# shijun18/H-DenseFormer

Measured on AMD Instinct MI355X. Metric: train samples/sec on 4x128^3 volumes, higher is better.
Workload: dtype bf16

## Files before the change

### h-denseformer_amd/csrc/conv_igemm.hip

```cpp
#include "conv_igemm.h"
#include "conv_tile.h"
#include <type_traits>

namespace {

template <typename T, int TD, int TH, int TW, int WM, int WN, int MB, int S, bool CONVT, bool FLAT = false>
__global__ __launch_bounds__(256, (FLAT && S == 1) ? 3 : 2) void conv_igemm_kernel(ConvArgs a) {
  if (a.prio) HDF_LIGHT_PRIO();
  static_assert(WM * WN == 4, "4 waves");
  static_assert(WM * MB * 32 == TD * TH * TW, "tile/wave decomposition");
  static_assert(!FLAT || TD == 1, "flat tiles are one voxel deep");
  constexpr int BD = FLAT ? 1 : (CONVT ? TD + 1 : S * (TD - 1) + 3);
  constexpr int BH = CONVT ? TH + 1 : S * (TH - 1) + 3;
  constexpr int BW = CONVT ? TW + 1 : S * (TW - 1) + 3;
  constexpr int SS = CONVT ? 1 : S;
  constexpr int ESZ = sizeof(T);
  __shared__ __attribute__((aligned(16))) char lds[BD * BH * BW * PITCH + 4 * 32 * 2 * 4];
  float* s_red = reinterpret_cast<float*>(lds + BD * BH * BW * PITCH);

  const int lane = threadIdx.x & 63, wave = threadIdx.x >> 6;
  const int r = lane & 31, h = lane >> 5;
  const int wm = wave / WN, wn = wave % WN;

  const int Td = CONVT ? a.Di : a.Do, Th = CONVT ? a.Hi : a.Ho, Tw = CONVT ? a.Wi : a.Wo;
  const int ntz = (Td + TD - 1) / TD, nty = (Th + TH - 1) / TH, ntx = (Tw + TW - 1) / TW;
  int t = blockIdx.x;
  const int tx = t % ntx;
  t /= ntx;
  const int ty = t % nty;
  t /= nty;
  const int tz = t % ntz;
  const int n = t / ntz;
  const int z0 = tz * TD, y0 = ty * TH, x0 = tx * TW;
  const int n_base = blockIdx.y * (WN * 32) + wn * 32;
  const int cls = CONVT ? blockIdx.z : 0;
  const int pz = FLAT ? 0 : (cls >> 2) & 1, py = (cls >> 1) & 1, px = cls & 1;
  const int ntapz = FLAT ? 1 : (CONVT ? (pz ? 2 : 1) : 3), ntapy = CONVT ? (py ? 2 : 1) : 3, ntapx = CONVT ? (px ? 2 : 1) : 3;

  const int oz = (CONVT || FLAT) ? z0 : S * z0 - 1, oy = CONVT ? y0 : S * y0 - 1, ox = CONVT ? x0 : S * x0 - 1;

  constexpr bool ZXMAP = !CONVT && !FLAT && S == 1 && TD == 4 && TW == 8 && WM * MB == TH && (2 * BH * BW) % 16 == 8;
  constexpr bool YXMAP = FLAT && SS == 1 && TW == 16 && 2 * WM * MB == TH;
  auto mrow_voxel = [](int mblk, int row, int& lz, int& ly, int& lx) {
    if constexpr (ZXMAP) {
      ws_row_to_zx(row, lz, lx);
      ly = mblk;
    } else if constexpr (YXMAP) {
      int g2;
      ds128_group(row, g2, lx);
      lz = 0;
      ly = 2 * mblk + g2;
    } else {
      const int lin = mblk * 32 + row;
      lz = lin / (TH * TW), ly = (lin / TW) % TH, lx = lin % TW;
    }
  };
  int rowbase[MB];
#pragma unroll
  for (int mb = 0; mb < MB; mb++) {
    int lz, ly, lx;
    mrow_voxel(wm * MB + mb, r, lz, ly, lx);
    rowbase[mb] = (((FLAT ? 0 : SS * lz)) * BH + SS * ly) * BW + SS * lx;
  }
  const bool n_active = n_base < a.CoutP;
  const char* wrow = reinterpret_cast<const char*>(a.w) + ((int64_t)(n_base + r) * a.Cin) * ESZ + h * 16;
  const int64_t wtap_stride = (int64_t)a.CoutP * a.Cin * ESZ;
  const int chunk_elems_max = 64 / ESZ;

  const char* const wfr = a.wfrag ? reinterpret_cast<const char*>(a.w) +
                                        (int64_t)(n_base >> 5) * ((a.Cin * ESZ) >> 5) * 1024 + r * 32 + h * 16
                                  : wrow;
  const int cstride = a.wfrag ? 2048 : 64, fstride = a.wfrag ? 1024 : 32;

  bool done = false;
  f32x16 acc[MB];
#pragma unroll
  for (int mb = 0; mb < MB; mb++)
#pragma unroll
    for (int i = 0; i < 16; i++) acc[mb][i] = 0.f;
  if constexpr (!CONVT) {
    if ((a.Cin * ESZ) % 64 == 0) {
      constexpr int NS = FLAT ? 18 : 54;
      constexpr int TAP0 = FLAT ? 9 : 0;
      constexpr int V1_RING_BIG = 6, V1_RING_SMALL = 9;
      constexpr int RING = (MB >= 4) ? V1_RING_BIG : V1_RING_SMALL;
      const int nchunk_all = a.Cin * ESZ / 64;
      const int kz = a.ksplit > 1 ? (int)blockIdx.z : 0;
      const int c_lo = a.ksplit > 1 ? kz * (nchunk_all / a.ksplit) : 0;
      const int nchunk = a.ksplit > 1 ? c_lo + nchunk_all / a.ksplit : nchunk_all;
      u32x4 bq[RING];
      auto b_load = [&](int chunk, int s_) -> u32x4 {
        const int tap = TAP0 + (s_ >> 1), fs = s_ & 1;
        const char* p = wfr + tap * wtap_stride + (int64_t)chunk * cstride + fs * fstride;
        return *reinterpret_cast<const u32x4*>(n_active ? p : reinterpret_cast<const char*>(a.w));
      };
      auto a_off = [&](int s_) {
        const int tap = s_ >> 1, fs = s_ & 1;
        return ((tap / 9 * BH + (tap / 3) % 3) * BW + tap % 3) * PITCH + h * 16 + fs * 32;
      };
#pragma unroll
      for (int k = 0; k < RING; k++) bq[k] = b_load(c_lo, k);
      for (int chunk = c_lo; chunk < nchunk; chunk++) {
        if (chunk > c_lo) __syncthreads();
        stage_box<T, BD, BH, BW, 64, PITCH>(lds, reinterpret_cast<const T*>(a.in), a.in_pitch, a.Cin, n, a.Di, a.Hi,
                                            a.Wi, oz, oy, ox, chunk * chunk_elems_max, 64, a.in_scale, a.in_shift,
                                            a.in_relu);
        __syncthreads();
        u32x4 af[2][MB];
#pragma unroll
        for (int mb = 0; mb < MB; mb++) af[0][mb] = *reinterpret_cast<const u32x4*>(lds + rowbase[mb] * PITCH + a_off(0));
        const bool more = chunk + 1 < nchunk;
#pragma unroll
        for (int s_ = 0; s_ < NS; s_++) {
          if (s_ + 1 < NS) {
#pragma unroll
            for (int mb = 0; mb < MB; mb++)
              af[(s_ + 1) & 1][mb] = *reinterpret_cast<const u32x4*>(lds + rowbase[mb] * PITCH + a_off(s_ + 1));
          }
          const u32x4 bcur = bq[s_ % RING];
          __builtin_amdgcn_sched_barrier(0);
#pragma unroll
          for (int mb = 0; mb < MB; mb++) Mma<T>::run(af[s_ & 1][mb], bcur, acc[mb]);
          if (s_ + RING < NS)
            bq[s_ % RING] = b_load(chunk, s_ + RING);
          else if (more)
            bq[s_ % RING] = b_load(chunk + 1, s_ + RING - NS);
          __builtin_amdgcn_sched_barrier(0);
        }
      }
      done = true;
    }
  }
  for (int c0 = 0; !done && c0 < a.Cin; c0 += chunk_elems_max) {
    const int chunk_elems = min(chunk_elems_max, a.Cin - c0);
    const int row_bytes = chunk_elems * ESZ;
    if (c0 > 0) __syncthreads();
    stage_box<T, BD, BH, BW, 64, PITCH>(lds, reinterpret_cast<const T*>(a.in), a.in_pitch, a.Cin, n, a.Di, a.Hi, a.Wi,
                                        oz, oy, ox, c0, row_bytes, a.in_scale, a.in_shift, a.in_relu);
    __syncthreads();
    if (n_active) {
      const int nfs = row_bytes >> 5;
      for (int jz = 0; jz < ntapz; jz++) {
        const int offz = FLAT ? 0 : (CONVT ? (pz ? 1 - jz : 0) : jz), wz = FLAT ? 1 : (CONVT ? (pz ? 2 * jz : 1) : jz);
        for (int jy = 0; jy < ntapy; jy++) {
          const int offy = CONVT ? (py ? 1 - jy : 0) : jy, wy = CONVT ? (py ? 2 * jy : 1) : jy;
#pragma unroll
          for (int jx = 0; jx < 3; jx++) {
            if (jx < ntapx) {
              const int offx = CONVT ? (px ? 1 - jx : 0) : jx, wx = CONVT ? (px ? 2 * jx : 1) : jx;
              const int tapoff = ((offz * BH + offy) * BW + offx) * PITCH + h * 16;
              const char* wp = wfr + ((wz * 3 + wy) * 3 + wx) * wtap_stride + (int64_t)(c0 * ESZ / 64) * cstride;
              for (int fs = 0; fs < nfs; fs++) {
                u32x4 bfrag = *reinterpret_cast<const u32x4*>(wp + fs * fstride);
                u32x4 afrag[MB];
#pragma unroll
                for (int mb = 0; mb < MB; mb++)
                  afrag[mb] = *reinterpret_cast<const u32x4*>(lds + rowbase[mb] * PITCH + tapoff + fs * 32);
#pragma unroll
                for (int mb = 0; mb < MB; mb++) Mma<T>::run(afrag[mb], bfrag, acc[mb]);
              }
            }
          }
        }
      }
    }
  }

  const int ch = n_base + r;
  if constexpr (!CONVT) {
    if (a.ksplit > 1) {
      if (n_active) {
        const int64_t mtot = (int64_t)a.N * a.Do * a.Ho * a.Wo;
#pragma unroll
        for (int mb = 0; mb < MB; mb++) {
#pragma unroll
          for (int i = 0; i < 16; i++) {
            const int row = (i & 3) + 8 * (i >> 2) + 4 * h;
            int lz, ly, lx;
            mrow_voxel(wm * MB + mb, row, lz, ly, lx);
            const int gz = z0 + lz, gy = y0 + ly, gx = x0 + lx;
            if (gz < Td && gy < Th && gx < Tw)
              a.kpart[((int64_t)blockIdx.z * mtot + (((int64_t)n * a.Do + gz) * a.Ho + gy) * a.Wo + gx) * a.CoutP + ch] =
                  acc[mb][i];
          }
        }
      }
      return;
    }
  }
  const bool ch_ok = n_active && ch < a.Cout;
  const float bias = (a.bias && ch_ok) ? a.bias[ch] : 0.f;
  float s1 = 0.f, s2 = 0.f;
  T* outp = (a.split && n_base >= a.split) ? reinterpret_cast<T*>(a.out2) - a.split : reinterpret_cast<T*>(a.out);
#pragma unroll
  for (int mb = 0; mb < MB; mb++) {
    float old[16];
    if (a.accumulate) {
#pragma unroll
      for (int i = 0; i < 16; i++) {
        int row = (i & 3) + 8 * (i >> 2) + 4 * h;
        int lz, ly, lx;
        mrow_voxel(wm * MB + mb, row, lz, ly, lx);
        int gz = z0 + lz, gy = y0 + ly, gx = x0 + lx;
        const bool ok = ch_ok && gz < Td && gy < Th && gx < Tw;
        int qz = (CONVT && !FLAT) ? 2 * gz + pz : gz, qy = CONVT ? 2 * gy + py : gy, qx = CONVT ? 2 * gx + px : gx;
        const T* p = outp + ((((int64_t)n * a.Do + qz) * a.Ho + qy) * a.Wo + qx) * a.out_pitch + ch;
        old[i] = ST<T>::ld(ok ? p : outp);
      }
    } else {
#pragma unroll
      for (int i = 0; i < 16; i++) old[i] = 0.f;
    }
#pragma unroll
    for (int i = 0; i < 16; i++) {
      int row = (i & 3) + 8 * (i >> 2) + 4 * h;
      int lz, ly, lx;
      mrow_voxel(wm * MB + mb, row, lz, ly, lx);
      int gz = z0 + lz, gy = y0 + ly, gx = x0 + lx;
      if (ch_ok && gz < Td && gy < Th && gx < Tw) {
        int qz = (CONVT && !FLAT) ? 2 * gz + pz : gz, qy = CONVT ? 2 * gy + py : gy, qx = CONVT ? 2 * gx + px : gx;
        T* p = outp + ((((int64_t)n * a.Do + qz) * a.Ho + qy) * a.Wo + qx) * a.out_pitch + ch;
        float v = acc[mb][i] + bias + old[i];
        ST<T>::st(p, v);
        s1 += v;
        s2 += v * v;
      }
    }
  }
  if (a.stat_partials) {
    s1 += __shfl_xor(s1, 32, 64);
    s2 += __shfl_xor(s2, 32, 64);
    __syncthreads();
    if (h == 0) {
      s_red[((wm * WN + wn) * 32 + r) * 2 + 0] = s1;
      s_red[((wm * WN + wn) * 32 + r) * 2 + 1] = s2;
    }
    __syncthreads();
    if (threadIdx.x < WN * 32) {
      int c = blockIdx.y * (WN * 32) + threadIdx.x;
      if (c < a.CoutP) {
        float t1 = 0.f, t2 = 0.f;
#pragma unroll
        for (int k = 0; k < WM; k++) {
          t1 += s_red[(k * WN * 32 + threadIdx.x) * 2 + 0];
          t2 += s_red[(k * WN * 32 + threadIdx.x) * 2 + 1];
        }
        float* q = a.stat_partials + ((int64_t)blockIdx.x * a.CoutP + c) * 2;
        q[0] = t1;
        q[1] = t2;
      }
    }
  }
}

template <int CH>
__device__ __forceinline__ int a_swz(int row) {
  return CH == 64 ? ((row >> 2) & 3) : ((row >> 3) & 1);
}

template <typename T, int CH, int RB, bool XF, int NB, bool BS = false, int TDP = 4>
__global__ __launch_bounds__(256) void conv_ws2_kernel(ConvArgs a) {
  if (a.prio) HDF_LIGHT_PRIO();
  constexpr int TD = TDP, ZH = TDP / 4, TH = 8, TW = 8, BD = TD + 2, BH = TH + 2, BW = TW + 2, BOX = BD * BH * BW;
  static_assert(TDP == 4 || TDP == 8, "tile depth");
  constexpr int ESZ = sizeof(T), EPC = ST<T>::EPC;
  constexpr int CIN = RB / ESZ;
  constexpr int NCH = RB / CH, NFS = CH / 32, NG = 9 * NFS;
  constexpr int CPV = CH / 16, CPV_SHIFT = (CPV == 4) ? 2 : 1;
  constexpr int TOTAL = BOX * CPV, NJ = (TOTAL + 255) / 256;
  constexpr bool SWZ = (2 * BOX * (CH + 16) + 4096 + 512 + 27 * 32 * NB * RB > 160 * 1024);
  constexpr int AP = SWZ ? CH : CH + 16;
  constexpr int ABUF = BOX * AP;
  constexpr int OFF_RED = 2 * ABUF, OFF_XF = OFF_RED + 2048 * NB, OFF_W = OFF_XF + 512;
  constexpr int NC = 32 * NB;
  constexpr int CPR = RB / 16, RP256 = 16 / CPR;
  static_assert(CH == 32 || CH == 64, "chunk bytes");
  static_assert(NCH == 1 || NCH % 2 == 0, "buffer parity at tile start must be compile-time");
  static_assert(2 * CIN * 4 <= 512, "scale/shift table");
  static_assert(OFF_W + 27 * NC * RB <= 160 * 1024, "LDS budget");
  static_assert(ZH == 1 || !SWZ, "the 8-deep tile needs the padded layout");
  __shared__ __attribute__((aligned(256))) char lds[OFF_W + 27 * NC * RB];
#ifdef WS_DBG_STAMPS
  const unsigned long long t_entry = __builtin_amdgcn_s_memrealtime();
#endif
  char* const a_lds = lds;
  float* const s_red = reinterpret_cast<float*>(lds + OFF_RED);
  float* const s_xf = reinterpret_cast<float*>(lds + OFF_XF);
  char* const w_lds = lds + OFF_W;

  const int tid = threadIdx.x, lane = tid & 63, wave = tid >> 6;
  const int r = lane & 31, h = lane >> 5;
  const int n0 = blockIdx.y * NC;
  const int part = tid & (CPV - 1);
  constexpr bool xf = XF;
  const float relu_lo = (xf && a.in_relu) ? 0.f : -INFINITY;

  {
    constexpr int WTOT = 27 * NC * CPR, WIT = (WTOT + 255) / 256;
    u32x4 wv[WIT];
    const int rot = blockIdx.x % WIT;
#pragma unroll
    for (int u = 0; u < WIT; u++) {
      int it = u + rot;
      it -= (it >= WIT) ? WIT : 0;
      const int id = min(tid + 256 * it, WTOT - 1);
      const int row = id / CPR, ch = id - row * CPR;
      const int tap = row / NC, rr = row - tap * NC;
      wv[u] = *reinterpret_cast<const u32x4*>(reinterpret_cast<const char*>(a.w) +
                                             ((int64_t)(tap * a.CoutP + n0 + rr) * CIN) * ESZ + ch * 16);
    }
#pragma unroll
    for (int u = 0; u < WIT; u++) {
      int it = u + rot;
      it -= (it >= WIT) ? WIT : 0;
      const int id = tid + 256 * it;
      const int row = id / CPR, ch = id - row * CPR;
      const int sw = ch ^ ((row / RP256) & (CPR - 1));
      if (id < WTOT) *reinterpret_cast<u32x4*>(w_lds + row * RB + sw * 16) = wv[u];
    }
  }
  const int bswz = (r / RP256) & (CPR - 1);

  const int ntz = (a.Do + TD - 1) / TD, nty = (a.Ho + TH - 1) / TH, ntx = (a.Wo + TW - 1) / TW;
  const bool has_int = ntz >= 3 && nty >= 3 && ntx >= 3;
  const int ipz = ntz - 2, ipy = nty - 2, ipx = ntx - 2;
  const int n_int = has_int ? a.N * ipz * ipy * ipx : 0;
  const int per_all = ntz * nty * ntx, per_bor = per_all - (has_int ? ipz * ipy * ipx : 0);
  const int n_bor = a.N * per_bor;
  const int G = gridDim.x;
  const int NX = (G % 8 == 0) ? 8 : 1;
  const int WPX = G / NX;
  const int xcd = blockIdx.x % NX, slot = blockIdx.x / NX;
  auto split = [&](int total, int& begin, int& cnt) {
    const int r0 = (int)((int64_t)total * xcd / NX), r1 = (int)((int64_t)total * (xcd + 1) / NX);
    begin = r0 + slot;
    cnt = (r1 - r0 > slot) ? (r1 - r0 - slot + WPX - 1) / WPX : 0;
  };
  int int_begin, int_cnt, bor_begin, bor_cnt;
  split(n_int, int_begin, int_cnt);
  split(n_bor, bor_begin, bor_cnt);
  if (int_cnt + bor_cnt == 0) return;
  int sdx = 0, sdy = 0, sdz = 0, sdn = 0;
  if (has_int) {
    int t = WPX;
    sdx = t % ipx, t /= ipx;
    sdy = t % ipy, t /= ipy;
    sdz = t % ipz, sdn = t / ipz;
  }

  int aaddr[SWZ ? 3 : 1][SWZ ? 4 : 1][SWZ ? 3 : 1];
  int abase;
  {
    int dz, x;
    ws_row_to_zx(r, dz, x);
    abase = ((dz * BH + 2 * wave) * BW + x) * AP + h * 16;
    if constexpr (SWZ) {
#pragma unroll
      for (int jz = 0; jz < 3; jz++)
#pragma unroll
        for (int yp = 0; yp < 4; yp++)
#pragma unroll
          for (int jx = 0; jx < 3; jx++) {
            int row = ((dz + jz) * BH + 2 * wave + yp) * BW + x + jx;
            aaddr[jz][yp][jx] = row * CH + ((h ^ a_swz<CH>(row)) << 4);
          }
    }
  }
  auto a_addr = [&](int jz, int yp, int jx, int fs, int zh = 0) {
    if constexpr (SWZ)
      return aaddr[jz][yp][jx] ^ (fs * 32);
    else
      return abase + (((jz + 4 * zh) * BH + yp) * BW + jx) * AP + fs * 32;
  };
  int bvar[NCH];
#pragma unroll
  for (int c = 0; c < NCH; c++) bvar[c] = r * RB + (((c * CPV + h) ^ bswz) << 4);
  int boff[NJ], bxyz[NJ], woff_t[SWZ ? NJ : 2];
#pragma unroll
  for (int j = 0; j < NJ; j++) {
    int vox = min(tid + 256 * j, TOTAL - CPV + part) >> CPV_SHIFT;
    int bz = vox / (BH * BW), rem = vox - bz * (BH * BW), by = rem / BW, bx = rem - by * BW;
    boff[j] = ((bz * a.Hi + by) * a.Wi + bx) * (int)a.in_pitch;
    bxyz[j] = (bz << 16) | (by << 8) | bx;
    if constexpr (SWZ) {
      woff_t[j] = vox * CH + ((part ^ a_swz<CH>(vox)) << 4);
    } else {
      if (j == 0) woff_t[0] = vox * AP + part * 16;
      if (j == NJ - 1) woff_t[1] = vox * AP + part * 16;
    }
  }
  auto woff = [&](int j) {
    if constexpr (SWZ)
      return woff_t[j];
    else
      return j == NJ - 1 ? woff_t[1] : woff_t[0] + j * (256 / CPV) * AP;
  };

  auto tile_lin = [&](const WsTile& c) { return ((c.n * ntz + c.z0 / TD) * nty + (c.y0 >> 3)) * ntx + (c.x0 >> 3); };
  auto int_init = [&](WsTile& c, int k) {
    int t = k;
    c.x0 = (t % ipx + 1) * TW;
    t /= ipx;
    c.y0 = (t % ipy + 1) * TH;
    t /= ipy;
    c.z0 = (t % ipz + 1) * TD;
    c.n = t / ipz;
    c.tile = tile_lin(c);
  };
  auto int_next = [&](WsTile& c) {
    int xi = (c.x0 >> 3) - 1 + sdx, yi = (c.y0 >> 3) - 1 + sdy, zi = c.z0 / TD - 1 + sdz;
    c.n += sdn;
    if (xi >= ipx) xi -= ipx, yi++;
    if (yi >= ipy) yi -= ipy, zi++;
    if (zi >= ipz) zi -= ipz, c.n++;
    c.x0 = (xi + 1) * TW, c.y0 = (yi + 1) * TH, c.z0 = (zi + 1) * TD;
    c.tile = tile_lin(c);
  };
  auto bor_init = [&](WsTile& c, int k) {
    int tz, ty, tx;
    c.k = k;
    c.n = k / per_bor;
    int rem = k - c.n * per_bor;
    if (!has_int) {
      tx = rem % ntx, ty = (rem / ntx) % nty, tz = rem / (ntx * nty);
    } else {
      const int plane = nty * ntx, ring = plane - ipy * ipx;
      if (rem < plane) {
        tz = 0, ty = rem / ntx, tx = rem % ntx;
      } else if (rem - plane < ipz * ring) {
        rem -= plane;
        tz = 1 + rem / ring;
        rem %= ring;
        if (rem < ntx) {
          ty = 0, tx = rem;
        } else if (rem - ntx < 2 * ipy) {
          rem -= ntx;
          ty = 1 + (rem >> 1), tx = (rem & 1) ? ntx - 1 : 0;
        } else {
          ty = nty - 1, tx = rem - ntx - 2 * ipy;
        }
      } else {
        rem -= plane + ipz * ring;
        tz = ntz - 1, ty = rem / ntx, tx = rem % ntx;
      }
    }
    c.z0 = tz * TD, c.y0 = ty * TH, c.x0 = tx * TW;
    c.tile = tile_lin(c);
  };
  auto bor_next = [&](WsTile& c) { bor_init(c, c.k + WPX); };
  auto tile_interior = [&](const WsTile& c) {
    return c.z0 >= 1 && c.y0 >= 1 && c.x0 >= 1 && c.z0 + TD + 1 <= a.Di && c.y0 + TH + 1 <= a.Hi &&
           c.x0 + TW + 1 <= a.Wi;
  };
  const T* const src_safe = reinterpret_cast<const T*>(a.in) + part * EPC;
  auto tile_org = [&](const WsTile& c) -> const T* {
    return src_safe + ((((int64_t)c.n * a.Di + (c.z0 - 1)) * a.Hi + (c.y0 - 1)) * a.Wi + (c.x0 - 1)) * a.in_pitch;
  };

  u32x4 pf[NJ];
  auto slot_ok = [&](int j, const WsTile& c) {
    int iz = c.z0 - 1 + (bxyz[j] >> 16), iy = c.y0 - 1 + ((bxyz[j] >> 8) & 255), ix = c.x0 - 1 + (bxyz[j] & 255);
    return ((unsigned)iz < (unsigned)a.Di) & ((unsigned)iy < (unsigned)a.Hi) & ((unsigned)ix < (unsigned)a.Wi);
  };
  auto load_one = [&](auto fast_tag, int j, int chunk, const WsTile& c, bool valid, bool inter, const T* org) {
    if constexpr (decltype(fast_tag)::value) {
      pf[j] = *reinterpret_cast<const u32x4*>(org + boff[j] + chunk * (CH / ESZ));
    } else {
      const bool ok = inter | (valid & slot_ok(j, c));
      const T* p = ok ? org + boff[j] + chunk * (CH / ESZ) : src_safe;
      pf[j] = *reinterpret_cast<const u32x4*>(p);
    }
  };
  float sc[EPC], sh[EPC];
  auto read_xf = [&](int chunk) {
    const int cb = chunk * (CH / ESZ) + part * EPC;
#pragma unroll
    for (int e = 0; e < EPC; e += 4) {
      f32x4 u = *reinterpret_cast<const f32x4*>(s_xf + cb + e);
      f32x4 v = *reinterpret_cast<const f32x4*>(s_xf + CIN + cb + e);
#pragma unroll
      for (int k = 0; k < 4; k++) {
        sc[e + k] = u[k];
        sh[e + k] = v[k];
      }
    }
  };
  auto commit_one = [&](auto fast_tag, int j, const WsTile& c, bool inter, char* dst) {
    u32x4 v = pf[j];
    if constexpr (XF) {
      float f[EPC];
      ST<T>::unpack(v, f);
#pragma unroll
      for (int e = 0; e < EPC; e++) f[e] = fmaxf(f[e] * sc[e] + sh[e], relu_lo);
      v = ST<T>::pack(f);
    }
    if constexpr (!decltype(fast_tag)::value) {
      const bool ok = inter | slot_ok(j, c);
#pragma unroll
      for (int k = 0; k < 4; k++) v[k] = ok ? v[k] : 0u;
    }
    *reinterpret_cast<u32x4*>(dst + woff(j)) = v;
  };
  int tbl_n = -1;
  auto refresh_xf = [&](int n) {
    if (tid < CIN) {
      s_xf[tid] = xf ? a.in_scale[(int64_t)n * CIN + tid] : 1.f;
      s_xf[CIN + tid] = xf ? a.in_shift[(int64_t)n * CIN + tid] : 0.f;
    }
    tbl_n = n;
    __syncthreads();
  };

  WsTile T0, T1, T2;
  bool v1 = false, v2 = false, i0 = false, i1 = false, i2 = false;
  const T *org0 = src_safe, *org1 = src_safe, *org2 = src_safe;
  int left = 0;
  auto begin_pass = [&](auto border_tag, int k, int count) __attribute__((always_inline)) {
    constexpr bool BORDER = decltype(border_tag)::value;
    auto next = [&](WsTile& c) {
      if constexpr (BORDER)
        bor_next(c);
      else
        int_next(c);
    };
    if constexpr (BORDER)
      bor_init(T0, k);
    else
      int_init(T0, k);
    left = count - 1;
    T1 = T0;
    next(T1);
// ... 149 lines not shown
              const float g = (yv[mb][i] * bsc + bsh > 0.f) ? ST<T>::ld(&tmp) : 0.f;
              s1 += g;
              s2 += g * ((yv[mb][i] - bmu) * brs);
            }
          }
          }
        } else {
#pragma unroll
        for (int zh = 0; zh < ZH; zh++)
#pragma unroll
        for (int mb = 0; mb < 2; mb++) {
          T* const orow = obase + (int64_t)mb * a.Wo * a.out_pitch + zh * ezh;
#pragma unroll
          for (int i = 0; i < 16; i++) {
            const float v = acc[(nb * ZH + zh) * 2 + mb][i] + bias[nb];
            ST<T>::st(orow + eoff(i), v);
            s1 += v;
            s2 += v * v;
          }
        }
        }
      } else if (full && ch_ok[nb]) {
#pragma unroll
        for (int zh = 0; zh < ZH; zh++)
#pragma unroll
        for (int mb = 0; mb < 2; mb++) {
          T* const orow = obase + (int64_t)mb * a.Wo * a.out_pitch + zh * ezh;
          float old[16];
#pragma unroll
          for (int i = 0; i < 16; i++) old[i] = ST<T>::ld(orow + eoff(i));
#pragma unroll
          for (int i = 0; i < 16; i++) {
            const float v = acc[(nb * ZH + zh) * 2 + mb][i] + bias[nb];
            ST<T>::st(orow + eoff(i), v + old[i]);
            s1 += v;
            s2 += v * v;
          }
        }
      } else {
#pragma unroll
        for (int zh = 0; zh < ZH; zh++)
#pragma unroll
        for (int mb = 0; mb < 2; mb++) {
          const int gy = y0 + 2 * wave + mb;
          T* const orow = obase + (int64_t)mb * a.Wo * a.out_pitch + zh * ezh;
#pragma unroll
          for (int i = 0; i < 16; i++) {
            const int gz = z0 + edz[i >> 2] + 4 * zh, gx = x0 + (i & 3) + 4 * ((i >> 2) & 1);
            const float v = acc[(nb * ZH + zh) * 2 + mb][i] + bias[nb];
            const bool ok = gz < a.Do && gy < a.Ho && gx < a.Wo;
            if (ok && ch_ok[nb]) {
              float o = v;
              if (a.accumulate) o += ST<T>::ld(orow + eoff(i));
              ST<T>::st(orow + eoff(i), o);
            }
            const float mk = ok ? 1.f : 0.f;
            s1 += mk * v;
            s2 += mk * v * v;
          }
        }
      }
      if (PLAIN || ch_ok[nb]) {
        lr1[nb] += s1;
        lr2[nb] += s2;
      }
    }
  };

  f32x16 acc[2 * NB * ZH];
  auto tile_phase = [&](auto par_tag, auto fast_tag, auto plain_tag) __attribute__((always_inline)) {
    constexpr int PAR0 = decltype(par_tag)::value;
#pragma unroll
    for (int c = 0; c < NCH; c++) {
      constexpr int dummy = 0;
      (void)dummy;
      const int PAR = (PAR0 + c) & 1;
      char* const a_rd = a_lds + PAR * ABUF;
      char* const a_wr = a_lds + (1 - PAR) * ABUF;
      const bool c_next = (c + 1 >= NCH);
      const int c_chunk = (c + 1) % NCH;
      const int l_tile = (c + 2) / NCH;
      const int l_chunk = (c + 2) % NCH;
      const WsTile& CT = c_next ? T1 : T0;
      const bool c_int = c_next ? (i1 | !v1) : i0;
      const WsTile& LT = l_tile == 0 ? T0 : (l_tile == 1 ? T1 : T2);
      const bool l_val = l_tile == 0 ? true : (l_tile == 1 ? v1 : v2);
      const bool l_int = l_tile == 0 ? i0 : (l_tile == 1 ? i1 : i2);
      const T* const l_org = l_tile == 0 ? org0 : (l_tile == 1 ? org1 : org2);
      WS2_STAMP(3)
      if constexpr (XF) {
        if (CT.n != tbl_n && (!c_next || v1)) refresh_xf(CT.n);
        read_xf(c_chunk);
      }
      WS2_STAMP(0)
      u32x4 af[2][4 * ZH], bf[2][3 * NB];
      const char* w_rd = w_lds;
      if constexpr (RB == 32) asm volatile("" : "+v"(w_rd));
      auto read_group = [&](int g, u32x4 (&A)[4 * ZH], u32x4 (&B)[3 * NB]) {
        const int t = g / NFS, fs = g % NFS, jz = t / 3, jx = t % 3;
        auto rdA = [&](int yp) {
#pragma unroll
          for (int zh = 0; zh < ZH; zh++) A[zh * 4 + yp] = *reinterpret_cast<const u32x4*>(a_rd + a_addr(jz, yp, jx, fs, zh));
        };
        auto rdB = [&](int jy) {
#pragma unroll
          for (int nb = 0; nb < NB; nb++)
            B[jy * NB + nb] = *reinterpret_cast<const u32x4*>(w_rd + ((jz * 9 + jy * 3 + jx) * NC + 32 * nb) * RB +
                                                              (bvar[c] ^ (fs * 32)));
        };
        rdB(0);
        rdA(0);
        rdA(1);
        rdB(1);
        rdA(2);
        rdB(2);
        rdA(3);
      };
      read_group(0, af[0], bf[0]);
#pragma unroll
      for (int g = 0; g < NG; g++) {
        if (g + 1 < NG) read_group(g + 1, af[(g + 1) & 1], bf[(g + 1) & 1]);
        __builtin_amdgcn_sched_barrier(0);
#pragma unroll
        for (int j = 0; j < NJ; j++) {
          if ((j * NG) / NJ == g) {
            commit_one(fast_tag, j, CT, c_int, a_wr);
            load_one(fast_tag, j, l_chunk, LT, l_val, l_int, l_org);
          }
        }
        u32x4(&A)[4 * ZH] = af[g & 1];
        u32x4(&B)[3 * NB] = bf[g & 1];
        if (c == 0 && g == 0) {
#pragma unroll
          for (int q2 = 0; q2 < 2 * NB * ZH; q2++)
#pragma unroll
            for (int i = 0; i < 16; i++) acc[q2][i] = 0.f;
        }
#pragma unroll
        for (int jy = 0; jy < 3; jy++)
#pragma unroll
          for (int nb = 0; nb < NB; nb++)
#pragma unroll
            for (int zh = 0; zh < ZH; zh++) {
              Mma<T>::run(A[zh * 4 + jy], B[jy * NB + nb], acc[(nb * ZH + zh) * 2 + 0]);
              Mma<T>::run(A[zh * 4 + jy + 1], B[jy * NB + nb], acc[(nb * ZH + zh) * 2 + 1]);
            }
        __builtin_amdgcn_sched_barrier(0);
      }
      WS2_STAMP(1)
      WS_BARRIER();
      WS2_STAMP(2)
    }
    epilogue(acc, T0, plain_tag);
    WS2_STAMP(4)
  };

  using P0 = std::integral_constant<int, 0>;
  using P1 = std::integral_constant<int, 1>;
  using Yes = std::true_type;
  using No = std::false_type;
  bool more = true;
  auto step = [&](auto border_tag) __attribute__((always_inline)) {
    constexpr bool BORDER = decltype(border_tag)::value;
    more = v1;
    if (!more) return;
    left--;
    T0 = T1;
    T1 = T2;
    i0 = i1;
    i1 = i2;
    v1 = v2;
    org0 = org1;
    org1 = org2;
    if constexpr (BORDER)
      bor_next(T2);
    else
      int_next(T2);
    v2 = left >= 2;
    i2 = v2 && (BORDER ? tile_interior(T2) : true);
    org2 = v2 ? tile_org(T2) : src_safe;
  };

  if (int_cnt > 0) {
    begin_pass(No{}, int_begin, int_cnt);
    more = true;
    int par = 0;
    if (plain) {
      while (more) {
        if (NCH > 1 || par == 0)
          tile_phase(P0{}, Yes{}, Yes{});
        else
          tile_phase(P1{}, Yes{}, Yes{});
        if (NCH == 1) par ^= 1;
        step(No{});
      }
    } else {
      while (more) {
        if (NCH > 1 || par == 0)
          tile_phase(P0{}, Yes{}, No{});
        else
          tile_phase(P1{}, Yes{}, No{});
        if (NCH == 1) par ^= 1;
        step(No{});
      }
    }
  }
  if (bor_cnt > 0) {
    begin_pass(Yes{}, bor_begin, bor_cnt);
    stats_to_row();
    cur_pass = 1;
    more = true;
    int par = 0;
    while (more) {
      if (NCH > 1 || par == 0)
        tile_phase(P0{}, No{}, No{});
      else
        tile_phase(P1{}, No{}, No{});
      if (NCH == 1) par ^= 1;
      step(Yes{});
    }
  }
  stats_to_row();
#ifdef WS_DBG_STAMPS
  if (tid == 0 && blockIdx.y == 0) {
    for (int k = 0; k < 5; k++) a.stat_partials[(int64_t)blockIdx.x * 8 + k] = (float)tacc[k];
    a.stat_partials[(int64_t)blockIdx.x * 8 + 5] = __uint_as_float((uint32_t)treal0);
    a.stat_partials[(int64_t)blockIdx.x * 8 + 6] = __uint_as_float((uint32_t)__builtin_amdgcn_s_memrealtime());
    a.stat_partials[(int64_t)blockIdx.x * 8 + 7] = (float)(__builtin_amdgcn_s_memtime() - tcyc0);
    a.stat_partials[2048 + blockIdx.x] = __uint_as_float((uint32_t)t_entry);
  }
#endif
}

template <typename T, int TD, int TH, int TW>
__global__ __launch_bounds__(256) void conv_ksplit_reduce_kernel(ConvArgs a) {
  if (a.prio) HDF_LIGHT_PRIO();
  __shared__ float red[16][64][2];
  const int ntz = (a.Do + TD - 1) / TD, nty = (a.Ho + TH - 1) / TH, ntx = (a.Wo + TW - 1) / TW;
  int t = blockIdx.x;
  const int tx = t % ntx;
  t /= ntx;
  const int ty = t % nty;
  t /= nty;
  const int tz = t % ntz, n = t / ntz;
  const int cl = ((int)threadIdx.x & 15) * 4, c0 = blockIdx.y * 64 + cl, vl = (int)threadIdx.x >> 4;
  const bool c_on = c0 < a.CoutP;
  const int64_t mtot = (int64_t)a.N * a.Do * a.Ho * a.Wo;
  float bias[4], s1[4] = {0.f, 0.f, 0.f, 0.f}, s2[4] = {0.f, 0.f, 0.f, 0.f};
#pragma unroll
  for (int e = 0; e < 4; e++) bias[e] = (a.bias && c0 + e < a.Cout) ? a.bias[c0 + e] : 0.f;
  constexpr int TV = TD * TH * TW, IT = (TV + 15) / 16;
  static_assert(TV % 16 == 0, "tile voxels per voxel lane");
  if (c_on) {
#pragma unroll 2
    for (int it = 0; it < IT; it++) {
      const int lin = vl + 16 * it;
      const int gz = tz * TD + lin / (TH * TW), gy = ty * TH + (lin / TW) % TH, gx = tx * TW + lin % TW;
      const bool ok = gz < a.Do && gy < a.Ho && gx < a.Wo;
      const int64_t vox = ok ? (((int64_t)n * a.Do + gz) * a.Ho + gy) * a.Wo + gx : 0;
      f32x4 pv[4];
#pragma unroll
      for (int k = 0; k < 4; k++)
        pv[k] = *reinterpret_cast<const f32x4*>(a.kpart + ((int64_t)min(k, a.ksplit - 1) * mtot + vox) * a.CoutP + c0);
      f32x4 v = pv[0];
      for (int k = 1; k < a.ksplit; k++) v += pv[k];
      if (ok) {
        T* p = reinterpret_cast<T*>(a.out) + vox * a.out_pitch + c0;
#pragma unroll
        for (int e = 0; e < 4; e++) {
          if (c0 + e < a.Cout) {
            float o = v[e] + bias[e];
            if (a.accumulate) o += ST<T>::ld(p + e);
            ST<T>::st(p + e, o);
            s1[e] += o;
            s2[e] += o * o;
          }
        }
      }
    }
  }
  if (a.stat_partials) {
#pragma unroll
    for (int e = 0; e < 4; e++) red[vl][cl + e][0] = s1[e], red[vl][cl + e][1] = s2[e];
    __syncthreads();
    if (threadIdx.x < 128) {
      const int c = threadIdx.x >> 1, j = threadIdx.x & 1;
      if (blockIdx.y * 64 + c < a.CoutP) {
        float sum = 0.f;
#pragma unroll
        for (int k = 0; k < 16; k++) sum += red[k][c][j];
        a.stat_partials[((int64_t)blockIdx.x * a.CoutP + blockIdx.y * 64 + c) * 2 + j] = sum;
      }
    }
  }
}

template <typename T, int TD, int TH, int TW, int WM, int WN, int MB, int S, bool CONVT, bool FLAT = false>
int launch_cfg(const ConvArgs& a0, hipStream_t st) {
  ConvArgs a = a0;
  const int Td = CONVT ? a.Di : a.Do, Th = CONVT ? a.Hi : a.Ho, Tw = CONVT ? a.Wi : a.Wo;
  const int tiles = a.N * ceil_div(Td, TD) * ceil_div(Th, TH) * ceil_div(Tw, TW), nblk = ceil_div(a.CoutP, WN * 32);
  a.ksplit = 1;
  if constexpr (!CONVT && S == 1) {
    const int nchunk = (a.Cin * (int)sizeof(T)) % 64 == 0 ? a.Cin * (int)sizeof(T) / 64 : 0;
    if (a.kpart && !a.split && a.CoutP <= 1024 && a.CoutP % 4 == 0 && a.out_pitch % 4 == 0) {
      for (int ks = 4; ks >= 2; ks >>= 1) {
        const size_t need = (size_t)ks * a.N * a.Do * a.Ho * a.Wo * a.CoutP * sizeof(float);
        if (tiles * nblk * ks <= hdf_cu_budget() && nchunk % ks == 0 && nchunk / ks >= 2 && need <= a.kpart_bytes) {
          a.ksplit = ks;
          break;
        }
      }
    }
  }
  dim3 grid(tiles, nblk, CONVT ? (FLAT ? 4 : 8) : a.ksplit);
  hipLaunchKernelGGL((conv_igemm_kernel<T, TD, TH, TW, WM, WN, MB, S, CONVT, FLAT>), grid, dim3(256), 0, st, a);
  HDF_LAUNCH_CHECK();
  if constexpr (!CONVT && S == 1) {
    if (a.ksplit > 1) {
      hipLaunchKernelGGL((conv_ksplit_reduce_kernel<T, TD, TH, TW>), dim3(tiles, ceil_div(a.CoutP, 64)), dim3(256), 0, st, a);
      HDF_LAUNCH_CHECK();
    }
  }
  return HDF_OK;
}

inline bool small_tile(int Do, int Ho, int Wo) {
  return (int64_t)Do * Ho * Wo <= 32 * 32 * 32 / 2;
}
inline bool tiny_tile(int Do, int Ho, int Wo) {
  return (int64_t)Do * Ho * Wo <= 8 * 8 * 16;
}
inline int ws_cfg(int mode, int Do, int Ho, int Wo, int row_bytes) {
  if (mode != 0 || row_bytes > 128 || (int64_t)Do * Ho * Wo < 48 * 48 * 48 || Do == 1) return 0;
  return (row_bytes == 32 || row_bytes == 64 || row_bytes == 128) ? 1 : 0;
}

template <typename T, int CH, int RB, int NB>
int launch_ws2(const ConvArgs& a, hipStream_t st) {
  const int budget = a.cu_budget > 0 ? std::min(a.cu_budget, hdf_cu_budget()) : hdf_cu_budget();
  const int cout_tiles = a.CoutP / (32 * NB);
#ifndef HDF_NO_WS2_TD8
  if constexpr (sizeof(T) == 2 && NB == 1 && RB == 64) {
    if (a.in_scale && !a.bs_y && a.Do % 8 == 0 && a.Do >= 24 && a.Ho >= 24 && a.Wo >= 24) {
      const int tiles8 = a.N * (a.Do / 8) * ceil_div(a.Ho, 8) * ceil_div(a.Wo, 8);
      const int gx8 = std::min(tiles8, std::max(1, budget / cout_tiles));
      hipLaunchKernelGGL((conv_ws2_kernel<T, CH, RB, true, NB, false, 8>), dim3(gx8, cout_tiles), dim3(256), 0, st, a);
      HDF_LAUNCH_CHECK();
      return HDF_OK;
    }
  }
#endif
  const int tiles = a.N * ceil_div(a.Do, 4) * ceil_div(a.Ho, 8) * ceil_div(a.Wo, 8);
  const int gx = std::min(tiles, std::max(1, budget / cout_tiles));
  if constexpr (sizeof(T) == 2 && NB == 1 && RB == 64) {
    if (a.bs_y && !a.in_scale) {
      hipLaunchKernelGGL((conv_ws2_kernel<T, CH, RB, false, NB, true>), dim3(gx, cout_tiles), dim3(256), 0, st, a);
      HDF_LAUNCH_CHECK();
      return HDF_OK;
    }
  }
  HDF_CHECK_ARG(a.bs_y == nullptr, "conv: backward statistics are not available for this launch (hdf_conv_bwd_stats_ok)");
  if (a.in_scale)
    hipLaunchKernelGGL((conv_ws2_kernel<T, CH, RB, true, NB>), dim3(gx, cout_tiles), dim3(256), 0, st, a);
  else
    hipLaunchKernelGGL((conv_ws2_kernel<T, CH, RB, false, NB>), dim3(gx, cout_tiles), dim3(256), 0, st, a);
  HDF_LAUNCH_CHECK();
  return HDF_OK;
}

inline int flat_tile(int Ho, int Wo) { return (int64_t)Ho * Wo <= 32 * 32 ? 0 : ((int64_t)Ho * Wo <= 64 * 64 ? 1 : 2); }

template <typename T>
int launch_conv_t(int mode, const ConvArgs& a, hipStream_t st) {
  if (a.Di == 1) {
    HDF_CHECK_ARG(a.Do == 1 && !a.bs_y, "conv: a depth-1 input selects the 2-D operator (output depth 1, no statistics epilogue of the 3-D data gradient)");
    if (mode == 0) {
      const int ft = flat_tile(a.Ho, a.Wo);
      if (ft == 0) return launch_cfg<T, 1, 8, 8, 2, 2, 1, 1, false, true>(a, st);
      if (ft == 1) return launch_cfg<T, 1, 8, 16, 2, 2, 2, 1, false, true>(a, st);
      if (a.CoutP <= 32) return launch_cfg<T, 1, 16, 16, 4, 1, 2, 1, false, true>(a, st);
      return launch_cfg<T, 1, 16, 16, 2, 2, 4, 1, false, true>(a, st);
    } else if (mode == 1) {
      if (a.CoutP <= 64) return launch_cfg<T, 1, 8, 8, 2, 2, 1, 2, false, true>(a, st);
      return launch_cfg<T, 1, 8, 8, 1, 4, 2, 2, false, true>(a, st);
    } else {
      if (hdf_convt_fused_takes(ST<T>::DT, a)) return hdf_launch_convt_fused(ST<T>::DT, a, st);
      if (a.CoutP <= 32) return launch_cfg<T, 1, 16, 16, 4, 1, 2, 1, true, true>(a, st);
      return launch_cfg<T, 1, 8, 16, 2, 2, 2, 1, true, true>(a, st);
    }
  }
  if (mode == 0) {
    const int rb = a.Cin * (int)sizeof(T);
    const int ws = ws_cfg(mode, a.Do, a.Ho, a.Wo, rb);
    if (ws) {
      if (rb == 32) return launch_ws2<T, 32, 32, 1>(a, st);
      if (rb == 64 && a.CoutP % 64 == 0) return launch_ws2<T, 32, 64, 2>(a, st);
      if (rb == 64) return launch_ws2<T, 32, 64, 1>(a, st);
      if (rb == 128) return launch_ws2<T, 32, 128, 1>(a, st);
    }
    if (tiny_tile(a.Do, a.Ho, a.Wo)) return launch_cfg<T, 2, 4, 8, 2, 2, 1, 1, false>(a, st);
    if (small_tile(a.Do, a.Ho, a.Wo)) return launch_cfg<T, 4, 4, 8, 2, 2, 2, 1, false>(a, st);
    if (a.CoutP <= 32) return launch_cfg<T, 4, 8, 8, 4, 1, 2, 1, false>(a, st);
    return launch_cfg<T, 4, 8, 8, 2, 2, 4, 1, false>(a, st);
  } else if (mode == 1) {
    if (hdf_conv_gather_s2_takes(ST<T>::DT, a)) return hdf_launch_conv_gather_s2(ST<T>::DT, a, st);
    if (a.CoutP <= 64) return launch_cfg<T, 2, 4, 8, 2, 2, 1, 2, false>(a, st);
    return launch_cfg<T, 4, 4, 4, 1, 4, 2, 2, false>(a, st);
  } else {
    if (hdf_convt_ws_takes(ST<T>::DT, a)) return hdf_launch_convt_ws(ST<T>::DT, a, st);
    if (hdf_convt_fused_takes(ST<T>::DT, a)) return hdf_launch_convt_fused(ST<T>::DT, a, st);
    if (a.CoutP <= 32) return launch_cfg<T, 4, 8, 8, 4, 1, 2, 1, true>(a, st);
    return launch_cfg<T, 4, 4, 8, 2, 2, 2, 1, true>(a, st);
  }
}

}

int hdf_conv_weight_layout(int dtype, int mode, int Cin, int Do, int Ho, int Wo) {
  const int rb = Cin * hdf_esz(dtype);
  if (rb % 64 != 0) return 0;
  if (Do == 1)
    return (mode == 2 && hdf_convt_fused_rows(rb)) ? 0 : 1;
  if (mode == 0) return ws_cfg(mode, Do, Ho, Wo, rb) ? 0 : 1;
  if (mode == 1) return 1;
  return hdf_convt_fused_rows(rb) ? 0 : 1;
}

bool hdf_conv_bwd_stats_ok(int dtype, const ConvArgs& a) {
  const int rb = a.Cin * hdf_esz(dtype);
  return dtype != HDF_F32 && rb == 64 && a.Cout == 32 && a.CoutP == 32 && !a.in_scale && !a.accumulate && !a.split &&
         a.Do % 4 == 0 && a.Ho % 8 == 0 && a.Wo % 8 == 0 && ws_cfg(0, a.Do, a.Ho, a.Wo, rb) && a.stat_partials &&
#ifndef HDF_NO_CONV_WR
         !hdf_conv_wr_takes(dtype, a) &&
#endif
         a.Di == a.Do && a.Hi == a.Ho && a.Wi == a.Wo;
}

int hdf_conv_stat_tiles(int mode, int Do, int Ho, int Wo, int row_bytes) {
  if (mode != 0) return 0;
  if (Do == 1) {
    const int ft = flat_tile(Ho, Wo);
    return ft == 0 ? ceil_div(Ho, 8) * ceil_div(Wo, 8) : (ft == 1 ? ceil_div(Ho, 8) * ceil_div(Wo, 16) : ceil_div(Ho, 16) * ceil_div(Wo, 16));
  }
  if (ws_cfg(mode, Do, Ho, Wo, row_bytes)) return WS_STAT_ROWS;
  if (tiny_tile(Do, Ho, Wo)) return ceil_div(Do, 2) * ceil_div(Ho, 4) * ceil_div(Wo, 8);
  if (small_tile(Do, Ho, Wo)) return ceil_div(Do, 4) * ceil_div(Ho, 4) * ceil_div(Wo, 8);
  return ceil_div(Do, 4) * ceil_div(Ho, 8) * ceil_div(Wo, 8);
}

int hdf_launch_conv(int dtype, int mode, const ConvArgs& a, hipStream_t st) {
  HDF_CHECK_ARG(a.Cin % 16 == 0, "conv: Cin=%d must be a multiple of 16 (pad the first layer)", a.Cin);
  HDF_CHECK_ARG(a.CoutP % 32 == 0 && a.CoutP >= a.Cout, "conv: bad CoutP=%d for Cout=%d", a.CoutP, a.Cout);
  HDF_CHECK_ARG(a.in_pitch % 8 == 0 && (((uintptr_t)a.in) & 15) == 0, "conv: input view must be 16-byte aligned");
  HDF_CHECK_ARG(mode == 0 || a.stat_partials == nullptr, "conv: stats only in mode 0");
  HDF_CHECK_ARG(a.wfrag == 0 || hdf_conv_weight_layout(dtype, mode, a.Cin, a.Do, a.Ho, a.Wo) == 1,
                "conv: fragment-major weights given to a launch that reads row-major panels (mode %d Cin %d)", mode, a.Cin);
  HDF_CHECK_ARG(a.split == 0 || (mode == 0 && a.split % 32 == 0 && a.split < a.Cout && a.out2 != nullptr),
                "conv: split output needs mode 0, split %% 32 == 0 and a second buffer (split=%d)", a.split);
#ifndef HDF_NO_CONV_WR
  if (mode == 0 && hdf_conv_wr_takes(dtype, a)) return hdf_launch_conv_wr(dtype, a, st);
#endif
  HDF_DISPATCH_T(dtype, return launch_conv_t<T>(mode, a, st));
  return HDF_ERR_UNSUPPORTED;
}
```

### h-denseformer_amd/csrc/conv_tile.h

```cpp
#pragma once
#include "hdf_common.h"

namespace {

template <typename T>
struct Mma;
template <>
struct Mma<bf16_t> {
  static __device__ __forceinline__ void run(const u32x4& a, const u32x4& b, f32x16& c) {
    c = __builtin_amdgcn_mfma_f32_32x32x16_bf16(__builtin_bit_cast(bf16x8, a), __builtin_bit_cast(bf16x8, b), c, 0, 0, 0);
  }
};
template <>
struct Mma<f16_t> {
  static __device__ __forceinline__ void run(const u32x4& a, const u32x4& b, f32x16& c) {
    c = __builtin_amdgcn_mfma_f32_32x32x16_f16(__builtin_bit_cast(f16x8, a), __builtin_bit_cast(f16x8, b), c, 0, 0, 0);
  }
};
template <>
struct Mma<float> {
  static __device__ __forceinline__ void run(const u32x4& a, const u32x4& b, f32x16& c) {
#pragma unroll
    for (int s = 0; s < 4; s++)
      c = __builtin_amdgcn_mfma_f32_32x32x2f32(__uint_as_float(a[s]), __uint_as_float(b[s]), c, 0, 0, 0);
  }
};

constexpr int PITCH = 80;

template <typename T, int BD, int BH, int BW, int ROWB , int LPITCH>
__device__ __forceinline__ void stage_box(char* lds, const T* __restrict__ src, int64_t pitch, int C, int n, int D,
                                          int H, int W, int oz, int oy, int ox, int c0, int row_bytes,
                                          const float* __restrict__ scale, const float* __restrict__ shift, int relu) {
  constexpr int EPC = ST<T>::EPC;
  const int cpv = row_bytes >> 4;
  const int cpv_shift = (cpv == 32) ? 5 : (cpv == 16) ? 4 : (cpv == 8) ? 3 : (cpv == 4) ? 2 : (cpv == 2) ? 1 : 0;
  const int total = (BD * BH * BW) << cpv_shift;
  const int part = threadIdx.x & (cpv - 1);
  const int cbase = c0 + part * EPC;
  float sc[EPC], sh[EPC];
  const bool xf = (scale != nullptr);
  if (xf) {
#pragma unroll
    for (int e = 0; e < EPC; e++) {
      bool ok = (cbase + e) < C;
      sc[e] = ok ? scale[(int64_t)n * C + cbase + e] : 0.f;
      sh[e] = ok ? shift[(int64_t)n * C + cbase + e] : 0.f;
    }
  }
  const bool chan_ok = cbase < C;
  constexpr int U = 5;
  for (int id0 = threadIdx.x; id0 < total; id0 += 256 * U) {
    u32x4 v[U];
    bool ok[U];
#pragma unroll
    for (int u = 0; u < U; u++) {
      int id = min(id0 + 256 * u, total - 1);
      int vox = id >> cpv_shift;
      int bz = vox / (BH * BW);
      int rem = vox - bz * (BH * BW);
      int by = rem / BW;
      int bx = rem - by * BW;
      int iz = oz + bz, iy = oy + by, ix = ox + bx;
      ok[u] = chan_ok && (unsigned)iz < (unsigned)D && (unsigned)iy < (unsigned)H && (unsigned)ix < (unsigned)W;
      const T* p = ok[u] ? src + ((((int64_t)n * D + iz) * H + iy) * W + ix) * pitch + cbase : src;
      v[u] = *reinterpret_cast<const u32x4*>(p);
    }
#pragma unroll
    for (int u = 0; u < U; u++) {
      int id = id0 + 256 * u;
      u32x4 w = v[u];
      if (xf) {
        float f[EPC];
        ST<T>::unpack(w, f);
#pragma unroll
        for (int e = 0; e < EPC; e++) {
          f[e] = f[e] * sc[e] + sh[e];
          if (relu) f[e] = fmaxf(f[e], 0.f);
        }
        w = ST<T>::pack(f);
      }
      if (!ok[u]) w = u32x4{0u, 0u, 0u, 0u};
      if (id < total) *reinterpret_cast<u32x4*>(lds + (id >> cpv_shift) * LPITCH + part * 16) = w;
    }
  }
}

constexpr int WS_STAT_ROWS = 512;
__device__ __forceinline__ void ds128_group(int r, int& g2, int& rank) {
  g2 = ((r >= 4 && r < 12) || (r >= 16 && r < 20) || r >= 28) ? 1 : 0;
  rank = g2 ? (r < 12 ? r - 4 : (r < 20 ? r - 8 : r - 16)) : (r < 4 ? r : (r < 16 ? r - 8 : r - 12));
}
__device__ __forceinline__ void ws_row_to_zx(int r, int& dz, int& x) {
  int g2, rank;
  ds128_group(r, g2, rank);
  dz = 2 * (rank >> 3) + g2;
  x = rank & 7;
}

#define WS_BARRIER()                                     \
  do {                                                   \
    asm volatile("s_waitcnt lgkmcnt(0)" ::: "memory");   \
    __builtin_amdgcn_s_barrier();                        \
    asm volatile("" ::: "memory");                       \
  } while (0)

struct WsTile {
  int n, z0, y0, x0, tile;
  int k;
};

__device__ __attribute__((aligned(16))) uint32_t g_zero_line[4] = {0u, 0u, 0u, 0u};

}

#ifdef WS_DBG_STAMPS
#define WS2_STAMP(k)                                       \
  {                                                        \
    __builtin_amdgcn_sched_barrier(0);                     \
    unsigned long long t_ = __builtin_amdgcn_s_memtime();  \
    __builtin_amdgcn_s_waitcnt(0xC07F);                    \
    __builtin_amdgcn_sched_barrier(0);                     \
    tacc[k] += t_ - tlast;                                 \
    tlast = t_;                                            \
  }
#else
#define WS2_STAMP(k)
#endif
```

Before: 186.8.

## Precompute halo-box offsets and prefetch next chunk's input slots across the MMA loop

Adds a BoxSlots helper that computes each thread's halo-box global offsets and bounds mask once per tile, so the per-chunk index arithmetic of stage_box disappears. For stride-1, non-flat bf16 tiles, the first few slots of the next channel chunk (and its scale/shift) are loaded into registers before the MMA loop runs, hiding global latency behind compute. It also replaces __syncthreads with a lighter lgkmcnt wait plus barrier and uses 32-bit offsets, falling back to the old path when a sample exceeds 2^30 elements. The cost is more VGPR pressure from the offset array and prefetch registers, which may reduce occupancy.

```diff
diff --git a/h-denseformer_amd/csrc/conv_igemm.hip b/h-denseformer_amd/csrc/conv_igemm.hip
--- a/h-denseformer_amd/csrc/conv_igemm.hip
+++ b/h-denseformer_amd/csrc/conv_igemm.hip
@@ -3,6 +3,19 @@
 #include <type_traits>
 
 namespace {
+
+__host__ __device__ constexpr int igemm_prefetch_slots(int esz, int MB, int S, bool FLAT, int NSLOT) {
+#ifdef HDF_IGEMM_PARENT_LOOP
+  return -1;
+#else
+  if (FLAT || S != 1 || MB < 2 || esz == 4) return -1;
+  if (MB >= 4) return NSLOT < 5 ? NSLOT : 5;
+  return NSLOT;
+#endif
+}
+__host__ __device__ inline bool igemm_sample_fits32(const ConvArgs& a) {
+  return (int64_t)a.Di * a.Hi * a.Wi * a.in_pitch < ((int64_t)1 << 30);
+}
 
 template <typename T, int TD, int TH, int TW, int WM, int WN, int MB, int S, bool CONVT, bool FLAT = false>
 __global__ __launch_bounds__(256, (FLAT && S == 1) ? 3 : 2) void conv_igemm_kernel(ConvArgs a) {
@@ -72,6 +85,10 @@
                                   : wrow;
   const int cstride = a.wfrag ? 2048 : 64, fstride = a.wfrag ? 1024 : 32;
 
+#ifdef WS_DBG_STAMPS
+  unsigned long long tacc[8] = {0, 0, 0, 0, 0, 0, 0, 0};
+  unsigned long long tlast = __builtin_amdgcn_s_memtime();
+#endif
   bool done = false;
   f32x16 acc[MB];
 #pragma unroll
@@ -79,7 +96,10 @@
 #pragma unroll
     for (int i = 0; i < 16; i++) acc[mb][i] = 0.f;
   if constexpr (!CONVT) {
-    if ((a.Cin * ESZ) % 64 == 0) {
+    using Box = BoxSlots<T, BD, BH, BW, PITCH>;
+    constexpr int NSLOT = Box::NSLOT;
+    constexpr int PF = igemm_prefetch_slots(sizeof(T), MB, S, FLAT, NSLOT);
+    if ((a.Cin * ESZ) % 64 == 0 && (PF < 0 || igemm_sample_fits32(a))) {
       constexpr int NS = FLAT ? 18 : 54;
       constexpr int TAP0 = FLAT ? 9 : 0;
       constexpr int V1_RING_BIG = 6, V1_RING_SMALL = 9;
@@ -100,16 +120,76 @@
       };
 #pragma unroll
       for (int k = 0; k < RING; k++) bq[k] = b_load(c_lo, k);
-      for (int chunk = c_lo; chunk < nchunk; chunk++) {
-        if (chunk > c_lo) __syncthreads();
-        stage_box<T, BD, BH, BW, 64, PITCH>(lds, reinterpret_cast<const T*>(a.in), a.in_pitch, a.Cin, n, a.Di, a.Hi,
-                                            a.Wi, oz, oy, ox, chunk * chunk_elems_max, 64, a.in_scale, a.in_shift,
-                                            a.in_relu);
-        __syncthreads();
+      WS2_STAMP(0);
+      constexpr int EPC = ST<T>::EPC, U = 5, PFN = PF > 0 ? PF : 0;
+      Box box;
+      const T* const src_n = reinterpret_cast<const T*>(a.in) + (int64_t)n * a.Di * a.Hi * a.Wi * a.in_pitch;
+      const bool xf = a.in_scale != nullptr;
+      const int64_t xoff = (int64_t)n * a.Cin + (threadIdx.x & 3) * EPC;
+      float sc[EPC], sh[EPC];
+      u32x4 pf[PFN > 0 ? PFN : 1];
+      auto load_xf = [&](int chunk, float (&s1)[EPC], float (&s2)[EPC]) {
+        if (xf) {
+#pragma unroll
+          for (int e = 0; e < EPC; e++) {
+            s1[e] = a.in_scale[xoff + chunk * chunk_elems_max + e];
+            s2[e] = a.in_shift[xoff + chunk * chunk_elems_max + e];
+          }
+        }
+      };
+      auto prefetch = [&](int chunk) {
+#pragma unroll
+        for (int u = 0; u < PFN; u++) pf[u] = box.load(u, src_n + chunk * chunk_elems_max);
+        if (PFN > 0) load_xf(chunk, sc, sh);
+      };
+      if constexpr (PF >= 0) {
+        box.init((int)a.in_pitch, a.Di, a.Hi, a.Wi, oz, oy, ox);
+        prefetch(c_lo);
+      }
+      for (int chunk_ = c_lo; chunk_ < nchunk; chunk_++) {
+        int chunk = chunk_;
+        if constexpr (PF >= 0) asm volatile("" : "+s"(chunk));
+        const bool more = chunk + 1 < nchunk;
+        if constexpr (PF < 0) {
+          if (chunk > c_lo) __syncthreads();
+          WS2_STAMP(2);
+          stage_box<T, BD, BH, BW, 64, PITCH>(lds, reinterpret_cast<const T*>(a.in), a.in_pitch, a.Cin, n, a.Di, a.Hi,
+                                              a.Wi, oz, oy, ox, chunk * chunk_elems_max, 64, a.in_scale, a.in_shift,
+                                              a.in_relu);
+          WS2_STAMP(1);
+          __syncthreads();
+          WS2_STAMP(2);
+        } else {
+          if (chunk > c_lo) WS_BARRIER();
+          WS2_STAMP(2);
+          const T* const src_c = src_n + chunk * chunk_elems_max;
+          float sc0[EPC], sh0[EPC];
+          if (PFN == 0) load_xf(chunk, sc0, sh0);
+          const float(&scr)[EPC] = PFN > 0 ? sc : sc0;
+          const float(&shr)[EPC] = PFN > 0 ? sh : sh0;
+          u32x4 v[U];
+#pragma unroll
+          for (int k = 0; k < U; k++)
+            if (PFN + k < NSLOT) v[k] = box.load(PFN + k, src_c);
+#pragma unroll
+          for (int u = 0; u < PFN; u++) box.commit(u, pf[u], lds, xf, scr, shr, a.in_relu);
+#pragma unroll
+          for (int u0 = PFN; u0 < NSLOT; u0 += U) {
+#pragma unroll
+            for (int k = 0; k < U; k++)
+              if (u0 + k < NSLOT) box.commit(u0 + k, v[k], lds, xf, scr, shr, a.in_relu);
+#pragma unroll
+            for (int k = 0; k < U; k++)
+              if (u0 + U + k < NSLOT) v[k] = box.load(u0 + U + k, src_c);
+          }
+          WS2_STAMP(1);
+          WS_BARRIER();
+          WS2_STAMP(2);
+          if (more) prefetch(chunk + 1);
+        }
         u32x4 af[2][MB];
 #pragma unroll
         for (int mb = 0; mb < MB; mb++) af[0][mb] = *reinterpret_cast<const u32x4*>(lds + rowbase[mb] * PITCH + a_off(0));
-        const bool more = chunk + 1 < nchunk;
 #pragma unroll
         for (int s_ = 0; s_ < NS; s_++) {
           if (s_ + 1 < NS) {
@@ -127,6 +207,7 @@
             bq[s_ % RING] = b_load(chunk + 1, s_ + RING - NS);
           __builtin_amdgcn_sched_barrier(0);
         }
+        WS2_STAMP(3);
       }
       done = true;
     }
@@ -227,6 +308,14 @@
       }
     }
   }
+#ifdef WS_DBG_STAMPS
+  WS2_STAMP(4);
+  if (a.stat_partials && threadIdx.x == 0 && blockIdx.y == 0 && blockIdx.z == 0) {
+    for (int k = 0; k < 5; k++) a.stat_partials[(int64_t)blockIdx.x * 8 + k] = (float)tacc[k];
+    a.stat_partials[(int64_t)blockIdx.x * 8 + 5] = (float)(a.Cin * ESZ / 64);
+  }
+  return;
+#endif
   if (a.stat_partials) {
     s1 += __shfl_xor(s1, 32, 64);
     s2 += __shfl_xor(s2, 32, 64);
@@ -982,7 +1071,7 @@
   const int tiles = a.N * ceil_div(Td, TD) * ceil_div(Th, TH) * ceil_div(Tw, TW), nblk = ceil_div(a.CoutP, WN * 32);
   a.ksplit = 1;
   if constexpr (!CONVT && S == 1) {
-    const int nchunk = (a.Cin * (int)sizeof(T)) % 64 == 0 ? a.Cin * (int)sizeof(T) / 64 : 0;
+    const int nchunk = ((a.Cin * (int)sizeof(T)) % 64 == 0 && igemm_sample_fits32(a)) ? a.Cin * (int)sizeof(T) / 64 : 0;
     if (a.kpart && !a.split && a.CoutP <= 1024 && a.CoutP % 4 == 0 && a.out_pitch % 4 == 0) {
       for (int ks = 4; ks >= 2; ks >>= 1) {
         const size_t need = (size_t)ks * a.N * a.Do * a.Ho * a.Wo * a.CoutP * sizeof(float);
diff --git a/h-denseformer_amd/csrc/conv_tile.h b/h-denseformer_amd/csrc/conv_tile.h
--- a/h-denseformer_amd/csrc/conv_tile.h
+++ b/h-denseformer_amd/csrc/conv_tile.h
@@ -86,6 +86,49 @@
   }
 }
 
+template <typename T, int BD, int BH, int BW, int LPITCH>
+struct BoxSlots {
+  static constexpr int EPC = ST<T>::EPC;
+  static constexpr int TOTAL = BD * BH * BW * 4;
+  static constexpr int NSLOT = (TOTAL + 255) / 256;
+  uint32_t off[NSLOT];
+  unsigned ok;
+  int lds0;
+  __device__ __forceinline__ void init(int pitch, int D, int H, int W, int oz, int oy, int ox) {
+    const int tid = threadIdx.x, part = tid & 3;
+    ok = 0u;
+    lds0 = (tid >> 2) * LPITCH + part * 16;
+#pragma unroll
+    for (int u = 0; u < NSLOT; u++) {
+      const int vox = min(tid + 256 * u, TOTAL - 1) >> 2;
+      const int bz = vox / (BH * BW), rem = vox - bz * (BH * BW), by = rem / BW, bx = rem - by * BW;
+      const int iz = oz + bz, iy = oy + by, ix = ox + bx;
+      const bool in = (unsigned)iz < (unsigned)D && (unsigned)iy < (unsigned)H && (unsigned)ix < (unsigned)W;
+      ok |= in ? (1u << u) : 0u;
+      off[u] = ((in ? (uint32_t)((iz * H + iy) * W + ix) * (uint32_t)pitch : 0u) + part * EPC) * (uint32_t)sizeof(T);
+    }
+  }
+  __device__ __forceinline__ u32x4 load(int u, const T* __restrict__ src_c) const {
+    return *reinterpret_cast<const u32x4*>(reinterpret_cast<const char*>(src_c) + off[u]);
+  }
+  __device__ __forceinline__ void commit(int u, u32x4 w, char* lds, bool xf, const float (&sc)[EPC], const float (&sh)[EPC],
+                                         int relu) const {
+    if (xf) {
+      float f[EPC];
+      ST<T>::unpack(w, f);
+#pragma unroll
+      for (int e = 0; e < EPC; e++) {
+        f[e] = f[e] * sc[e] + sh[e];
+        if (relu) f[e] = fmaxf(f[e], 0.f);
+      }
+      w = ST<T>::pack(f);
+    }
+    if (!((ok >> u) & 1u)) w = u32x4{0u, 0u, 0u, 0u};
+    if ((u + 1) * 256 <= TOTAL || (int)threadIdx.x + 256 * u < TOTAL)
+      *reinterpret_cast<u32x4*>(lds + lds0 + u * 64 * LPITCH) = w;
+  }
+};
+
 constexpr int WS_STAT_ROWS = 512;
 __device__ __forceinline__ void ds128_group(int r, int& g2, int& rank) {
   g2 = ((r >= 4 && r < 12) || (r >= 16 && r < 20) || r >= 28) ? 1 : 0;
```

Result: no change. 187.0 (median of 2 runs) (+0.1%).
